# AKGWSB/EzRT

Hardware: NVIDIA H100
Metric: Mrays/s (primary+secondary) (higher is better)
Workload: dtype f32

## Files before the change

ezrt_b200/csrc/device_functions.cuh:

```cuda
#ifndef EZRT_DEVICE_FUNCTIONS_CUH
#define EZRT_DEVICE_FUNCTIONS_CUH

#include "device_scene.h"
#include "ezrt.h"
#include "ezrt_math.h"
#include "w8_node.h"

__constant__ uint32_t c_sobolV[8 * 32] = {
#include "ezrt_sobol_table.inc"
};

typedef ez_vec3 vec3;

__device__ __forceinline__ vec3 f4xyz(float4 q) { return ez_v3(q.x, q.y, q.z); }
__device__ __forceinline__ vec3 splat3(float s) { return ez_v3(s, s, s); }
__device__ __forceinline__ float4 ldg4(const float4* p) { return __ldg(p); }

#ifndef EZRT_MATH_NOINLINE
#define EZRT_MATH_NOINLINE 0
#endif
#if EZRT_MATH_NOINLINE
#define EZD_MATH __device__ __noinline__
#else
#define EZD_MATH __device__ __forceinline__
// ... 711 lines not shown
                        if (strict) {
                            best = tn;
                            best_tri = leaf_first + __ffs(mq) - 1;
                        }
                        if (ANYHIT && (!BOUNDED || strict)) stop = true;
                    }
                    leaf_first += LL;
                    leaf_cnt -= LL;
                }
                if (long_leaves) m_leaf |= __ballot_sync(FULL, pos >= 0 && leaf_cnt > 0 && !stop);
            }
            if (at_leaf) {
                ref = EZRT_REF_DONE;
                if (!stop) {
                    while (sp > 0) {
                        const int2 e = STACK_POP();
                        if (PRUNE && prune_test(__int_as_float(e.y), best, slack)) continue;
                        ref = e.x;
                        break;
                    }
                }
            }
            if (ray >= 0 && ref == EZRT_REF_DONE) {
                HitRec h;
                h.t = best;
                h.tri = best_tri;
                float ix, iy, iz, iz2;
                pk2_split(rs.inv_xy, ix, iy);
                pk2_split(rs.inv_zz, iz, iz2);
                io.store((uint32_t)ray, h, tie, o, d, ez_v3(ix, iy, iz));
                ray = -1;
            }
            busy = __ballot_sync(FULL, ray >= 0);
        } while (busy != 0u && (exhausted || __popc(busy) >= refill_thresh));
    }
    if (COUNT) {
        atomicAdd(counts.node_visits, n_visits);
        atomicAdd(counts.tri_tests, n_tests);
    }
}

#undef STACK_PUSH
#undef STACK_POP

__device__ __forceinline__ uint32_t prmt(uint32_t a, uint32_t b, uint32_t sel) {
    uint32_t r;
    asm("prmt.b32 %0, %1, %2, %3;" : "=r"(r) : "r"(a), "r"(b), "r"(sel));
    return r;
}
template <int K>
__device__ __forceinline__ float w8_plane(uint32_t w, uint32_t bias) {
    uint32_t r;
    asm("prmt.b32 %0, %1, %2, %3;" : "=r"(r) : "r"(w), "r"(bias), "n"(0x7604 | (K << 4)));
    return __uint_as_float(r);
}
template <int K>
__device__ __forceinline__ bool w8_slot_hit(uint32_t nx, uint32_t ny, uint32_t nz, uint32_t fx, uint32_t fy, uint32_t fz, float Bx, float By, float Bz,
                                            float Ax, float Ay, float Az, float limit, uint32_t bias) {
    const float tnx = __fmaf_rn(w8_plane<K>(nx, bias), Bx, Ax), tny = __fmaf_rn(w8_plane<K>(ny, bias), By, Ay), tnz = __fmaf_rn(w8_plane<K>(nz, bias), Bz, Az);
    const float tfx = __fmaf_rn(w8_plane<K>(fx, bias), Bx, Ax), tfy = __fmaf_rn(w8_plane<K>(fy, bias), By, Ay), tfz = __fmaf_rn(w8_plane<K>(fz, bias), Bz, Az);
    const float tmin = fmaxf(fmaxf(tnx, tny), fmaxf(tnz, 0.0f));
    const float tmax = fminf(fminf(tfx, tfy), fminf(tfz, limit));
    return tmin <= tmax;
}

__device__ __forceinline__ int nth_set_bit(uint32_t m, int r) {
    int pos = 0, c = __popc(m & 0xffffu);
    if (r >= c) { r -= c; m >>= 16; pos += 16; }
    c = __popc(m & 0xffu);
    if (r >= c) { r -= c; m >>= 8; pos += 8; }
    c = __popc(m & 0xfu);
    if (r >= c) { r -= c; m >>= 4; pos += 4; }
    c = __popc(m & 0x3u);
    if (r >= c) { r -= c; m >>= 2; pos += 2; }
    return pos + ((r >= (int)(m & 1u)) ? 1 : 0);
}

__device__ __forceinline__ uint32_t w8_clock() {
    uint32_t t;
    asm volatile("mov.u32 %0, %%clock;" : "=r"(t) : : "memory");
    return t;
}

#define W8_ENDED (-2)
template <bool ANYHIT, bool COUNT, bool IDX, bool BOUNDED = false, class RayIO>
__device__ __forceinline__ void extend_w8(const SceneDev& sc, uint32_t n, uint32_t* work, RayIO io, const unsigned char* s_perm, uint2* stack_sm,
                                          W8Counts counts, unsigned long long* phase_cycles) {
    const bool tri_na = sc.tri_l1_bypass != 0;
    const int refill_thresh = sc.refill_thresh, leaf_thresh = sc.w8_tri_weight;
    const unsigned FULL = 0xffffffffu;
    const int lane = threadIdx.x & 31;
    const unsigned lt_mask = (1u << lane) - 1u;
    const int stack_stride = blockDim.x;
    const int stack_cap = sc.w8_stack_entries;
    uint2 stack_local[W8_LOCAL_STACK];
    uint2* const my_stack = stack_sm + threadIdx.x;
    const uint4* __restrict__ nodes = sc.w8_nodes;
    const float origin_limit = sc.w8_origin_limit, inv_limit = sc.quant_inv_limit;
    const uint32_t bias = sc.w8_decode_bits;
    __shared__ unsigned char s_owner_all[EZRT_EXTEND_MAX_THREADS];
    unsigned char* const s_owner = s_owner_all + (threadIdx.x & ~31u);

    int ray = -1;
    int node = -1;
    int end_leaf = 0;
    int sp = 0;
    vec3 o = splat3(0.0f), d = splat3(0.0f), inv = splat3(0.0f);
    float slack = 0.0f, best = EZ_INF;
    int best_tri = -1;
    bool tie = false;
    uint32_t near_mask = 0;
    uint32_t g_base = 0, g_bits = 0;
    uint32_t t_base = 0, t_mask = 0;
    uint32_t n_visits = 0, n_tests = 0;
    uint32_t cyc_refill = 0, cyc_node = 0, cyc_tri = 0, cyc_end = 0;
    uint32_t end_dt = 0, t_mark = COUNT ? w8_clock() : 0u;
    bool exhausted = false;
    uint32_t chunk_pos = 0, chunk_end = 0;
    const uint32_t chunk = (uint32_t)sc.work_chunk;

#define W8_PUSH(e) do { const uint2 e__ = (e); if (sp < stack_cap) my_stack[sp * stack_stride] = e__; else stack_local[sp - stack_cap] = e__; ++sp; } while (0)
#define W8_POP() ((--sp < stack_cap) ? my_stack[sp * stack_stride] : stack_local[sp - stack_cap])
    auto select_next = [&]() {
        if ((g_bits >> 8) == 0u) {
            if (sp == 0) {
                const uint32_t te = COUNT ? w8_clock() : 0u;
                if (best_tri >= 0) end_leaf = io.leaf_of(best_tri);
                if (COUNT) end_dt = w8_clock() - te;
                node = W8_ENDED;
                return;
            }
            const uint2 e = W8_POP();
            g_base = e.x;
            g_bits = e.y;
        }
        const int p = 23 - __clz(g_bits);
        g_bits ^= 0x100u << p;
        const uint32_t slot = (uint32_t)p ^ near_mask;
        node = (int)(g_base + __popc(g_bits & 0xffu & ((1u << slot) - 1u)));
    };

    while (true) {
        const bool ended = node == W8_ENDED;
        const unsigned need = __ballot_sync(FULL, ray < 0 || ended);
        const bool claim = need != 0u && !exhausted && chunk_pos >= chunk_end;
        uint32_t base = 0;
        if (claim && lane == 0) base = atomicAdd(work, chunk);
        if (ended) {
            HitRec h;
            h.t = best;
            h.tri = best_tri;
            const uint32_t te = COUNT ? w8_clock() : 0u;
            io.finish((uint32_t)ray, h, tie, o, d, inv, end_leaf);
            if (COUNT) end_dt = w8_clock() - te;
            ray = -1;
            node = -1;
        }
        if (need != 0u && !exhausted) {
            if (claim) {
                base = __shfl_sync(FULL, base, 0);
                chunk_pos = base;
                chunk_end = (base + chunk < n) ? base + chunk : n;
                if (base >= n) exhausted = true;
            }
            if (!exhausted && ray < 0) {
                uint32_t idx = chunk_pos + (uint32_t)__popc(need & lt_mask);
                if (idx < chunk_end && io.load(idx, o, d)) {
                    inv = ez_v3(EZ_DIV(1.0f, d.x), EZ_DIV(1.0f, d.y), EZ_DIV(1.0f, d.z));
                    const float ax = ez_abs(inv.x), ay = ez_abs(inv.y), az = ez_abs(inv.z);
                    const float ao = fmaxf(ez_abs(o.x), fmaxf(ez_abs(o.y), ez_abs(o.z)));
                    const float amin = fminf(ax, fminf(ay, az)), amax = fmaxf(ax, fmaxf(ay, az));
                    if ((amax <= inv_limit) && (amin >= W8_INV_MIN) && (ao <= origin_limit)) {
                        slack = sc.prune_delta * ez_max(ax, ez_max(ay, az));
                        near_mask = (d.x >= 0.0f ? (1u << sc.w8_near_bit[0]) : 0u) | (d.y >= 0.0f ? (1u << sc.w8_near_bit[1]) : 0u) |
                                    (d.z >= 0.0f ? (1u << sc.w8_near_bit[2]) : 0u);
                        ray = (int)idx;
                        node = 0;
                        sp = 0;
                        g_bits = 0u;
                        t_mask = 0u;
                        best = ray_tmax<BOUNDED>(io, idx);
                        best_tri = -1;
                        tie = false;
                    } else {
                        io.defer(idx, o, d);
                    }
                }
            }
            if (!exhausted) {
                uint32_t take = (uint32_t)__popc(need);
                chunk_pos = (chunk_pos + take < chunk_end) ? chunk_pos + take : chunk_end;
            }
        }
        if (COUNT) {
            const uint32_t now = w8_clock(), e = __reduce_max_sync(FULL, end_dt);
            end_dt = 0u;
            cyc_end += e;
            cyc_refill += now - t_mark - e;
            t_mark = now;
        }
        if (__ballot_sync(FULL, ray >= 0) == 0u) {
            if (exhausted) break;
            continue;
        }
        const int tri_weight = leaf_thresh;
        unsigned busy;
        do {
            const bool at_node = node >= 0;
            const unsigned m_node = __ballot_sync(FULL, at_node);
            const uint32_t pairs = __reduce_add_sync(FULL, (uint32_t)__popc(t_mask));
            if (m_node == 0u && pairs == 0u) { busy = 0u; break; }
            const bool node_step = m_node != 0u && tri_weight * (int)min(pairs, 32u) < __popc(m_node);
            if (node_step) {
                if (at_node) {
                    const uint4* nd = nodes + (size_t)node * (W8_NODE_WORDS / 4);
                    const uint4 h = ldg128_u32(nd), c = ldg128_u32(nd + 1), l = ldg128_u32(nd + 2), m = ldg128_u32(nd + 3), u = ldg128_u32(nd + 4);
                    if (COUNT) n_visits++;
                    const float limit = best + (best * 0.000244140625f + slack);
                    const float Bx = __uint_as_float(W8_SCALE_BITS(h.w, 0)) * inv.x, By = __uint_as_float(W8_SCALE_BITS(h.w, 1)) * inv.y,
                                Bz = __uint_as_float(W8_SCALE_BITS(h.w, 2)) * inv.z;
                    const float Ax = __fmaf_rn(-W8_DECODE_BIAS, Bx, (__uint_as_float(h.x) - o.x) * inv.x);
                    const float Ay = __fmaf_rn(-W8_DECODE_BIAS, By, (__uint_as_float(h.y) - o.y) * inv.y);
                    const float Az = __fmaf_rn(-W8_DECODE_BIAS, Bz, (__uint_as_float(h.z) - o.z) * inv.z);
                    const bool px = d.x >= 0.0f, py = d.y >= 0.0f, pz = d.z >= 0.0f;
                    const uint32_t nx0 = px ? c.z : m.z, nx1 = px ? c.w : m.w, fx0 = px ? m.z : c.z, fx1 = px ? m.w : c.w;
                    const uint32_t ny0 = py ? l.x : u.x, ny1 = py ? l.y : u.y, fy0 = py ? u.x : l.x, fy1 = py ? u.y : l.y;
                    const uint32_t nz0 = pz ? l.z : u.z, nz1 = pz ? l.w : u.w, fz0 = pz ? u.z : l.z, fz1 = pz ? u.w : l.w;
                    uint32_t hits = 0u;
                    if (w8_slot_hit<0>(nx0, ny0, nz0, fx0, fy0, fz0, Bx, By, Bz, Ax, Ay, Az, limit, bias)) hits |= 1u;
                    if (w8_slot_hit<1>(nx0, ny0, nz0, fx0, fy0, fz0, Bx, By, Bz, Ax, Ay, Az, limit, bias)) hits |= 2u;
                    if (w8_slot_hit<2>(nx0, ny0, nz0, fx0, fy0, fz0, Bx, By, Bz, Ax, Ay, Az, limit, bias)) hits |= 4u;
                    if (w8_slot_hit<3>(nx0, ny0, nz0, fx0, fy0, fz0, Bx, By, Bz, Ax, Ay, Az, limit, bias)) hits |= 8u;
                    if (w8_slot_hit<0>(nx1, ny1, nz1, fx1, fy1, fz1, Bx, By, Bz, Ax, Ay, Az, limit, bias)) hits |= 16u;
                    if (w8_slot_hit<1>(nx1, ny1, nz1, fx1, fy1, fz1, Bx, By, Bz, Ax, Ay, Az, limit, bias)) hits |= 32u;
                    if (w8_slot_hit<2>(nx1, ny1, nz1, fx1, fy1, fz1, Bx, By, Bz, Ax, Ay, Az, limit, bias)) hits |= 64u;
                    if (w8_slot_hit<3>(nx1, ny1, nz1, fx1, fy1, fz1, Bx, By, Bz, Ax, Ay, Az, limit, bias)) hits |= 128u;
                    const uint32_t imask = h.w >> 24;
                    const uint32_t inner = hits & imask;
                    uint32_t leaf = hits & ~imask;
                    if ((g_bits >> 8) != 0u) W8_PUSH(make_uint2(g_base, g_bits));
                    g_base = c.x;
                    g_bits = imask | ((uint32_t)s_perm[near_mask * 256u + inner] << 8);
                    t_base = c.y;
                    t_mask = 0u;
                    while (leaf != 0u) {
                        const int s = __ffs(leaf) - 1;
                        leaf &= leaf - 1u;
                        const uint32_t mb = ((s < 4 ? m.x : m.y) >> ((s & 3) * 8)) & 0xffu;
                        t_mask |= ((1u << (mb >> 5)) - 1u) << (mb & 31u);
                    }
                    node = -1;
                    if (t_mask == 0u) select_next();
                }
            } else {
                const uint32_t cnt = (uint32_t)__popc(t_mask);
                uint32_t incl = cnt;
#pragma unroll
                for (int s = 1; s < 32; s <<= 1) {
                    const uint32_t v = __shfl_up_sync(FULL, incl, s);
                    if (lane >= s) incl += v;
                }
                const uint32_t first = incl - cnt;
                const bool owns = cnt != 0u && first < 32u;
                const unsigned starts = __reduce_or_sync(FULL, owns ? 1u << first : 0u);
                __syncwarp();
                if (owns) s_owner[first] = (unsigned char)lane;
                __syncwarp();
                const int start = 31 - __clz(starts & (FULL >> (31 - lane)));
                const bool act = (uint32_t)lane < pairs;
                const int src = act ? (int)s_owner[start] : lane;
                vec3 ro, rd;
                ro.x = __shfl_sync(FULL, o.x, src); ro.y = __shfl_sync(FULL, o.y, src); ro.z = __shfl_sync(FULL, o.z, src);
                rd.x = __shfl_sync(FULL, d.x, src); rd.y = __shfl_sync(FULL, d.y, src); rd.z = __shfl_sync(FULL, d.z, src);
                const float rbest = __shfl_sync(FULL, best, src);
                const uint32_t rmask = __shfl_sync(FULL, t_mask, src);
// ... 843 lines not shown
```

ezrt_b200/csrc/kernels.cu:

```cuda
#include "kernels.h"

#include <cstdlib>
#include <map>
#include <mutex>

#include "device_functions.cuh"

__device__ __forceinline__ void in_tile_xy(int in_tile, int& ix, int& iy) {
    int sub = in_tile >> 5, lane = in_tile & 31;
    ix = (sub & 1) * 8 + (lane & 7);
    iy = (sub >> 1) * 4 + (lane >> 3);
}
__device__ __forceinline__ bool slot_pixel(const RenderDev& rd, const TileDev* __restrict__ tiles, uint32_t slot,
                                           uint32_t& px, uint32_t& py, uint32_t& frame_in_batch) {
    uint32_t per_frame = (uint32_t)rd.n_tiles * EZRT_TILE_PIXELS;
    frame_in_batch = slot / per_frame;
    uint32_t r = slot - frame_in_batch * per_frame;
    TileDev t = tiles[r >> 8];
    int ix, iy;
    in_tile_xy((int)(r & 255u), ix, iy);
    px = (uint32_t)(t.x0 + ix);
    py = (uint32_t)(t.y0 + iy);
    return ix < t.w && iy < t.h;
}
// ... 142 lines not shown
    PathQueue q;
    const uint32_t* perm;
    const uint32_t* to_accel;
    float2* side_hit;
    __device__ __forceinline__ bool load(uint32_t i, vec3& o, vec3& d) const {
        const uint32_t j = perm ? perm[i] : i;
        float4 o4 = __ldcs(q.ray_o + j), d4 = __ldcs(q.ray_d + j);
        o = ez_v3(o4.x, o4.y, o4.z);
        d = ez_v3(d4.x, d4.y, d4.z);
        return true;
    }
    __device__ __forceinline__ void store(uint32_t i, HitRec h, bool, vec3, vec3, vec3) const {
        const uint32_t j = perm ? perm[i] : i;
        int tri = h.tri;
        if (to_accel && tri >= 0) tri = (int)__ldg(to_accel + tri);
        if (side_hit) side_hit[i] = make_float2(h.t, __int_as_float(tri));
        else __stcs(q.hit + j, make_float2(h.t, __int_as_float(tri)));
    }
    __device__ __forceinline__ void defer(uint32_t, vec3, vec3) const {}
};

template <bool PRUNE, bool ANYHIT>
__global__ void __launch_bounds__(EZRT_EXTEND_MAX_THREADS, EZRT_EXTEND_LB_BLOCKS) k_extend(SceneDev sc, PathQueue q, const uint32_t* __restrict__ q_count,
                                                                uint32_t* work, const uint32_t* __restrict__ perm, int to_accel, float2* side_hit, int gate) {
    ExtendIO io;
    io.q = q;
    io.perm = perm;
    io.to_accel = to_accel ? sc.ref_to_acc : nullptr;
    io.side_hit = side_hit;
    const uint32_t n = *q_count;
    if (blockIdx.x * blockDim.x >= n) return;
    if ((gate == 1 && n > EZRT_SIDE_CAP) || (gate == 2 && n <= EZRT_SIDE_CAP)) return;
    TreeView tree = reference_tree(sc);
    if (gate == 1) tree.top_nodes = 0;
    stage_top_nodes(tree);
    extend_persistent<PRUNE, ANYHIT, false, false, 8, false, false>(sc, tree, n, work, io, g_smem_top);
}


struct ShadowIO {
    ShadowQueue sq;
    float4* Lo;
    const uint32_t* perm;
    __device__ __forceinline__ bool load(uint32_t i, vec3& o, vec3& d) const {
        const uint32_t j = perm ? perm[i] : i;
        float4 o4 = __ldcs(sq.ray_o + j), d4 = __ldcs(sq.ray_d + j);
        o = ez_v3(o4.x, o4.y, o4.z);
        d = ez_v3(d4.x, d4.y, d4.z);
        return true;
    }
    __device__ __forceinline__ void mark(uint32_t j, bool lit) const { sq.lit[j] = lit ? 1 : 0; }
    __device__ __forceinline__ float tmax(uint32_t i) const { return __ldcs(sq.nrm + (perm ? perm[i] : i)).w; }
    __device__ __forceinline__ void store(uint32_t i, HitRec h, bool, vec3, vec3, vec3) const { mark(perm ? perm[i] : i, h.tri < 0); }
    __device__ __forceinline__ void defer(uint32_t, vec3, vec3) const {}
};

template <bool PRUNE, bool BOUNDED = false>
__global__ void __launch_bounds__(EZRT_EXTEND_MAX_THREADS, EZRT_EXTEND_LB_BLOCKS) k_shadow(SceneDev sc, ShadowQueue sq, const uint32_t* __restrict__ s_count,
                                                                uint32_t* work, float4* __restrict__ Lo, const uint32_t* __restrict__ perm) {
    ShadowIO io;
    io.sq = sq;
    io.Lo = Lo;
    io.perm = perm;
    const uint32_t n = *s_count;
    if (blockIdx.x * blockDim.x >= n) return;
    const TreeView tree = reference_tree(sc);
    stage_top_nodes(tree);
    extend_persistent<PRUNE, true, false, false, 8, false, false, BOUNDED>(sc, tree, n, work, io, g_smem_top);
}

__device__ __forceinline__ void w8_smem_setup(unsigned char*& s_perm, uint2*& stack_sm) {
    unsigned char* base = reinterpret_cast<unsigned char*>(g_smem_top);
    s_perm = base;
    stack_sm = reinterpret_cast<uint2*>(base + 2048);
    for (int i = threadIdx.x; i < 2048; i += blockDim.x) {
        const int m = i >> 8, x = i & 255;
        int y = 0;
        for (int b = 0; b < 8; b++)
            if ((x >> b) & 1) y |= 1 << (b ^ m);
        s_perm[i] = (unsigned char)y;
    }
    __syncthreads();
}

struct AccelExtendIO {
    PathQueue q;
    const int* acc_tri_leaf;
    const float4* leaf_box;
    uint32_t* defer_list;
    uint32_t* defer_count;
    const uint32_t* perm;
    __device__ __forceinline__ bool load(uint32_t i, vec3& o, vec3& d) const {
        const uint32_t j = perm ? perm[i] : i;
        float4 o4 = __ldcs(q.ray_o + j), d4 = __ldcs(q.ray_d + j);
        o = ez_v3(o4.x, o4.y, o4.z);
        d = ez_v3(d4.x, d4.y, d4.z);
        return true;
    }
    __device__ __forceinline__ void defer(uint32_t i, vec3, vec3) const {
        const uint32_t j = perm ? perm[i] : i;
        __stcs(q.hit + j, make_float2(0.0f, __int_as_float(EZRT_TRI_PENDING)));
        defer_list[atomicAdd(defer_count, 1u)] = j;
    }
    __device__ __forceinline__ void store(uint32_t i, HitRec h, bool tie, vec3 o, vec3 d, vec3 inv) const {
        if (h.tri >= 0 && (tie || !reference_reaches_leaf_inv(acc_tri_leaf, leaf_box, h.tri, o, inv))) {
            defer(i, o, d);
            return;
        }
        __stcs(q.hit + (perm ? perm[i] : i), make_float2(h.t, __int_as_float(h.tri)));
    }
    __device__ __forceinline__ int leaf_of(int tri) const { return __ldg(acc_tri_leaf + tri); }
    __device__ __forceinline__ void finish(uint32_t i, HitRec h, bool tie, vec3 o, vec3 d, vec3 inv, int leaf) const {
        if (h.tri >= 0 && (tie || !reference_reaches_leaf_box(leaf_box, leaf, o, inv))) {
            defer(i, o, d);
            return;
        }
        __stcs(q.hit + (perm ? perm[i] : i), make_float2(h.t, __int_as_float(h.tri)));
    }
};

struct AccelCameraIO {
    RenderDev rd;
    const TileDev* tiles;
    uint32_t batch_first_frame;
    uint32_t n_frames;
    uint32_t per_frame;
    PathQueue q;
    const int* acc_tri_leaf;
    const float4* leaf_box;
    uint32_t* defer_list;
    uint32_t* defer_count;
    __device__ __forceinline__ uint32_t slot_of(uint32_t i) const {
        if (n_frames == 0u) return i;
        const uint32_t p = i / n_frames;
        return (i - p * n_frames) * per_frame + p;
    }
    __device__ __forceinline__ bool load(uint32_t i, vec3& o, vec3& d) const {
        uint32_t px, py, fib, seed;
        if (!slot_pixel(rd, tiles, slot_of(i), px, py, fib)) return false;
        primary_ray(rd, px, py, batch_first_frame + fib, seed, o, d);
        return true;
    }
    __device__ __forceinline__ void defer_slot(uint32_t slot, vec3 o, vec3 d) const {
        q.ray_o[slot] = make_float4(o.x, o.y, o.z, 0.0f);
        q.ray_d[slot] = make_float4(d.x, d.y, d.z, 0.0f);
        __stcs(q.hit + slot, make_float2(0.0f, __int_as_float(EZRT_TRI_PENDING)));
        defer_list[atomicAdd(defer_count, 1u)] = slot;
    }
    __device__ __forceinline__ void defer(uint32_t i, vec3 o, vec3 d) const { defer_slot(slot_of(i), o, d); }
    __device__ __forceinline__ void store(uint32_t i, HitRec h, bool tie, vec3 o, vec3 d, vec3 inv) const {
        const uint32_t slot = slot_of(i);
        if (h.tri >= 0 && (tie || !reference_reaches_leaf_inv(acc_tri_leaf, leaf_box, h.tri, o, inv))) {
            defer_slot(slot, o, d);
            return;
        }
        __stcs(q.hit + slot, make_float2(h.t, __int_as_float(h.tri)));
    }
};

template <bool COUNT, bool IDX>
__global__ void __launch_bounds__(EZRT_EXTEND_MAX_THREADS, EZRT_EXTEND_LB_BLOCKS) k_extend_w8_camera(SceneDev sc, RenderDev rd, const TileDev* __restrict__ tiles,
                                                                   uint32_t batch_first_frame, uint32_t n_slots, uint32_t n_frames, PathQueue q, uint32_t* work,
                                                                   uint32_t* defer_list, uint32_t* defer_count, W8Counts counts) {
    unsigned char* s_perm;
    uint2* stack_sm;
    w8_smem_setup(s_perm, stack_sm);
    AccelCameraIO io;
    io.rd = rd;
    io.tiles = tiles;
    io.batch_first_frame = batch_first_frame;
    io.n_frames = n_frames;
    io.per_frame = (uint32_t)rd.n_tiles * EZRT_TILE_PIXELS;
    io.q = q;
    io.acc_tri_leaf = sc.acc_tri_leaf;
    io.leaf_box = sc.leaf_box;
    io.defer_list = defer_list;
    io.defer_count = defer_count;
    extend_w8_bundle<COUNT, IDX>(sc, n_slots, work, io, s_perm, stack_sm, counts);
}

template <bool COUNT, bool IDX>
__global__ void __launch_bounds__(EZRT_EXTEND_MAX_THREADS, EZRT_EXTEND_LB_BLOCKS) k_extend_w8(SceneDev sc, PathQueue q, const uint32_t* __restrict__ q_count, uint32_t* work,
                                                                   uint32_t* defer_list, uint32_t* defer_count, W8Counts counts, const uint32_t* __restrict__ perm,
                                                                   unsigned long long* phase_cycles) {
    unsigned char* s_perm;
    uint2* stack_sm;
    w8_smem_setup(s_perm, stack_sm);
    AccelExtendIO io;
    io.q = q;
    io.acc_tri_leaf = sc.acc_tri_leaf;
    io.leaf_box = sc.leaf_box;
    io.defer_list = defer_list;
    io.defer_count = defer_count;
    io.perm = perm;
    extend_w8<false, COUNT, IDX>(sc, *q_count, work, io, s_perm, stack_sm, counts, phase_cycles);
}

struct AccelShadowIO {
    ShadowIO base;
    const int* acc_tri_leaf;
    const float4* leaf_box;
    uint32_t* defer_list;
    uint32_t* defer_count;
    __device__ __forceinline__ bool load(uint32_t i, vec3& o, vec3& d) const { return base.load(i, o, d); }
    __device__ __forceinline__ float tmax(uint32_t i) const { return base.tmax(i); }
    __device__ __forceinline__ void defer(uint32_t i, vec3, vec3) const { defer_list[atomicAdd(defer_count, 1u)] = i; }
    __device__ __forceinline__ void store(uint32_t i, HitRec h, bool, vec3 o, vec3 d, vec3 inv) const {
        if (h.tri < 0) {
            base.mark(i, true);
            return;
        }
        if (!reference_reaches_leaf_inv(acc_tri_leaf, leaf_box, h.tri, o, inv)) defer(i, o, d);
        else base.mark(i, false);
    }
    __device__ __forceinline__ int leaf_of(int tri) const { return __ldg(acc_tri_leaf + tri); }
    __device__ __forceinline__ void finish(uint32_t i, HitRec h, bool, vec3 o, vec3 d, vec3 inv, int leaf) const {
        if (h.tri < 0) base.mark(i, true);
        else if (!reference_reaches_leaf_box(leaf_box, leaf, o, inv)) defer(i, o, d);
        else base.mark(i, false);
    }
};

template <bool COUNT, bool IDX, bool BOUNDED = false>
__global__ void __launch_bounds__(EZRT_EXTEND_MAX_THREADS, EZRT_EXTEND_LB_BLOCKS) k_shadow_w8(SceneDev sc, ShadowQueue sq, const uint32_t* __restrict__ s_count, uint32_t* work,
                                                                   float4* __restrict__ Lo, uint32_t* defer_list, uint32_t* defer_count, W8Counts counts,
                                                                   unsigned long long* phase_cycles) {
    unsigned char* s_perm;
    uint2* stack_sm;
    w8_smem_setup(s_perm, stack_sm);
    AccelShadowIO io;
    io.base.sq = sq;
    io.base.Lo = Lo;
    io.base.perm = nullptr;
    io.acc_tri_leaf = sc.acc_tri_leaf;
    io.leaf_box = sc.leaf_box;
    io.defer_list = defer_list;
    io.defer_count = defer_count;
    extend_w8<true, COUNT, IDX, BOUNDED>(sc, *s_count, work, io, s_perm, stack_sm, counts, phase_cycles);
}

template <bool COUNT, bool Q16>
__global__ void __launch_bounds__(EZRT_EXTEND_MAX_THREADS, EZRT_EXTEND_LB_BLOCKS) k_extend_accel(SceneDev sc, PathQueue q, const uint32_t* __restrict__ q_count, uint32_t* work,
                                                                      uint32_t* defer_list, uint32_t* defer_count, W8Counts counts, const uint32_t* __restrict__ perm) {
    AccelExtendIO io;
    io.q = q;
    io.acc_tri_leaf = sc.acc_tri_leaf;
    io.leaf_box = sc.leaf_box;
    io.defer_list = defer_list;
    io.defer_count = defer_count;
    io.perm = perm;
    extend_persistent<true, false, true, true, 4, COUNT, Q16>(sc, accel_tree(sc), *q_count, work, io, g_smem_top, counts);
}
template <bool COUNT>
__global__ void __launch_bounds__(EZRT_EXTEND_MAX_THREADS, EZRT_EXTEND_LB_BLOCKS) k_extend_accel_camera(SceneDev sc, RenderDev rd, const TileDev* __restrict__ tiles,
                                                                      uint32_t batch_first_frame, uint32_t n_slots, uint32_t n_frames, PathQueue q, uint32_t* work,
                                                                      uint32_t* defer_list, uint32_t* defer_count, W8Counts counts) {
    AccelCameraIO io;
    io.rd = rd;
    io.tiles = tiles;
    io.batch_first_frame = batch_first_frame;
    io.n_frames = n_frames;
    io.per_frame = (uint32_t)rd.n_tiles * EZRT_TILE_PIXELS;
    io.q = q;
    io.acc_tri_leaf = sc.acc_tri_leaf;
    io.leaf_box = sc.leaf_box;
    io.defer_list = defer_list;
    io.defer_count = defer_count;
    extend_persistent<true, false, true, true, 4, COUNT, false>(sc, accel_tree(sc), n_slots, work, io, g_smem_top, counts, sc.refill_thresh_camera, sc.work_chunk_camera);
}
template <bool COUNT, bool Q16, bool BOUNDED = false>
__global__ void __launch_bounds__(EZRT_EXTEND_MAX_THREADS, EZRT_EXTEND_LB_BLOCKS) k_shadow_accel(SceneDev sc, ShadowQueue sq, const uint32_t* __restrict__ s_count, uint32_t* work,
                                                                      float4* __restrict__ Lo, uint32_t* defer_list, uint32_t* defer_count, W8Counts counts) {
    AccelShadowIO io;
    io.base.sq = sq;
    io.base.Lo = Lo;
    io.base.perm = nullptr;
    io.acc_tri_leaf = sc.acc_tri_leaf;
    io.leaf_box = sc.leaf_box;
    io.defer_list = defer_list;
    io.defer_count = defer_count;
    extend_persistent<true, true, true, true, 4, COUNT, Q16, BOUNDED>(sc, accel_tree(sc), *s_count, work, io, g_smem_top, counts);
}

#ifndef EZRT_SHADE_REGROUP
#define EZRT_SHADE_REGROUP 0
#endif
#define EZRT_SOBOL_TABLE 256
#define EZRT_SHADE_KEYS 18
#ifndef EZRT_SHADE_PREFETCH
#define EZRT_SHADE_PREFETCH 0
#endif
#ifndef EZRT_SHADE_MIN_BLOCKS
#define EZRT_SHADE_MIN_BLOCKS 8
#endif
template <int MODE, bool LIST, bool AOV = false, bool ENV = false, bool TRANS = false>
__global__ void __launch_bounds__(128, EZRT_SHADE_MIN_BLOCKS) k_shade(SceneDev sc, RenderDev rd, const TileDev* __restrict__ tiles, int bounce,
                                               uint32_t batch_first_frame, PathQueue qin, const uint32_t* __restrict__ in_count,
                                               PathQueue qout, uint32_t* out_count, ShadowQueue sq, uint32_t* s_count,
                                               float4* __restrict__ Lo, float4* __restrict__ Le, uint32_t n_fused, uint32_t n_frames,
                                               const uint32_t* __restrict__ list, const float2* __restrict__ side_hit,
                                               float4* __restrict__ aov_rec, LightsDev lights, EnvDev env) {
    __shared__ float2 s_sobol[EZRT_SOBOL_TABLE];
    const bool sobol_table = (MODE == EZRT_MODE_DISNEY_SOBOL_P5 || MODE == EZRT_MODE_DISNEY_IS_MIS_P5 || MODE == EZRT_MODE_DISNEY_LIGHTS) &&
                             n_frames <= EZRT_SOBOL_TABLE;
    if (sobol_table) {
        for (uint32_t f = threadIdx.x; f < n_frames; f += blockDim.x) s_sobol[f] = sobol_pair(bounce, batch_first_frame + f);
        __syncthreads();
    }
    __shared__ uint32_t s_scan[34];
    const uint32_t n = (LIST || !n_fused) ? *in_count : n_fused;
    if (LIST && n > EZRT_SIDE_CAP) return;
    const uint32_t n_round = ((n + blockDim.x - 1u) / blockDim.x) * blockDim.x;
    const uint32_t stride = gridDim.x * blockDim.x;
#if EZRT_SHADE_REGROUP
    __shared__ float4 s_rg[4][128];
    __shared__ float2 s_rg_hit[128];
    __shared__ unsigned short s_rg_cnt[4][2];
#endif
    for (uint32_t i0 = blockIdx.x * blockDim.x + threadIdx.x; i0 < n_round; i0 += stride) {
        uint32_t i = i0;
#if EZRT_SHADE_PREFETCH
// ... 503 lines not shown
                    const size_t q = (size_t)qy * width + qx;
                    cq = cv_in[q];
                    const float4 aq0 = aov[2 * q];
                    if (aq0.w == 0.0f || !ez_finite(cq.x) || !ez_finite(cq.y) || !ez_finite(cq.z) || !ez_finite(cq.w)) continue;
                    const float4 aq1 = aov[2 * q + 1];
                    const int d = max(abs(i), abs(j));
                    w = ez_atrous_weight(h, (float)(step * d), n_p, ez_v3(aq1.x, aq1.y, aq1.z), ap1.w, aq1.w, Y_p, ez_luminance(ez_v3(cq.x, cq.y, cq.z)),
                                         sd_p, a_p, ez_v3(aq0.x, aq0.y, aq0.z), sigma_l, sigma_n, sigma_z, sigma_a);
                }
                sw = sw + w;
                sc = ez_add(sc, ez_scale(ez_v3(cq.x, cq.y, cq.z), w));
                sv = sv + (w * w) * cq.w;
            }
        }
        res = make_float4(EZ_DIV(sc.x, sw), EZ_DIV(sc.y, sw), EZ_DIV(sc.z, sw), EZ_DIV(sv, sw * sw));
    }
    if (out) {
        const size_t o = p * (size_t)channels;
        if (channels == 4) out[o + 3] = color_in[o + 3];
        out[o] = res.x; out[o + 1] = res.y; out[o + 2] = res.z;
    } else {
        cv_out[p] = res;
    }
}

static inline int div_up(long long a, long long b) { return (int)((a + b - 1) / b); }

static int extend_threads() {
    static int v = 0;
    if (v == 0) {
        v = EZRT_EXTEND_THREADS;
        if (const char* e = getenv("EZRT_EXTEND_THREADS")) v = std::max(32, std::min(EZRT_EXTEND_MAX_THREADS, (atoi(e) / 32) * 32));
    }
    return v;
}
static int extend_blocks_per_sm() {
    static int v = 0;
    if (v == 0) {
        v = EZRT_EXTEND_BLOCKS_PER_SM;
        if (const char* e = getenv("EZRT_EXTEND_BPS")) v = std::max(1, std::min(16, atoi(e)));
    }
    return v;
}
void launch_generate(const RenderDev& rd, const TileDev* tiles, uint32_t n_slots, uint32_t batch_first_frame, PathQueue q,
                     uint32_t* q_count, int n_sms, cudaStream_t st) {
    int blocks = std::min(div_up(n_slots, 256), n_sms * 8);
    k_generate<<<blocks, 256, 0, st>>>(rd, tiles, n_slots, batch_first_frame, q, q_count);
}
static void set_dynamic_smem(const void* kernel, size_t bytes) {
    static std::mutex mu;
    static std::map<const void*, size_t> done;
    std::lock_guard<std::mutex> lock(mu);
    auto it = done.find(kernel);
    if (it != done.end() && it->second >= bytes) return;
    cudaFuncSetAttribute(kernel, cudaFuncAttributeMaxDynamicSharedMemorySize, (int)bytes);
    done[kernel] = bytes;
}
template <class K>
static size_t smem_for(K kernel, int top_nodes) {
    size_t bytes = (size_t)top_nodes * EZRT_TOP_STRIDE * sizeof(float4) + (size_t)EZRT_SMEM_STACK * sizeof(int2) * extend_threads();
    set_dynamic_smem((const void*)kernel, std::max<size_t>(bytes, 1024));
    return bytes;
}
static int persistent_blocks(uint32_t n_max, int n_sms) {
    int blocks = std::min(div_up(n_max, extend_threads()), n_sms * extend_blocks_per_sm());
    return blocks < 1 ? 1 : blocks;
}

void launch_extend(const SceneDev& sc, bool prune, bool anyhit, PathQueue q, const uint32_t* q_count, uint32_t* work,
                   const uint32_t* perm, int to_accel, uint32_t n_max, int n_sms, cudaStream_t st, float2* side_hit, int gate) {
    int threads = extend_threads(), blocks = persistent_blocks(n_max, n_sms);
    int top = sc.top_nodes;
    if (gate == 1) {
        threads = 128;
        blocks = std::max(1, std::min(div_up(n_max, threads), 64));
        top = 0;
    }
    if (prune && anyhit) k_extend<true, true><<<blocks, threads, smem_for(k_extend<true, true>, top), st>>>(sc, q, q_count, work, perm, to_accel, side_hit, gate);
    else if (prune) k_extend<true, false><<<blocks, threads, smem_for(k_extend<true, false>, top), st>>>(sc, q, q_count, work, perm, to_accel, side_hit, gate);
    else if (anyhit) k_extend<false, true><<<blocks, threads, smem_for(k_extend<false, true>, top), st>>>(sc, q, q_count, work, perm, to_accel, side_hit, gate);
    else k_extend<false, false><<<blocks, threads, smem_for(k_extend<false, false>, top), st>>>(sc, q, q_count, work, perm, to_accel, side_hit, gate);
}
template <class K>
static size_t w8_smem_for(K kernel, const SceneDev& sc) {
    size_t bytes = 2048 + (size_t)sc.w8_stack_entries * sizeof(uint2) * extend_threads();
    set_dynamic_smem((const void*)kernel, bytes);
    return bytes;
}
void launch_extend_accel(const SceneDev& sc, PathQueue q, const uint32_t* q_count, uint32_t* work, uint32_t* defer_list,
                         uint32_t* defer_count, uint32_t* defer_work, uint32_t n_max, int n_sms, unsigned long long* counts, const uint32_t* perm,
                         cudaStream_t st, int exact_gate) {
    const int threads = extend_threads(), blocks = persistent_blocks(n_max, n_sms);
    if (sc.w8_nodes) {
        W8Counts c;
        c.node_visits = counts ? counts + 2 : nullptr;
        c.tri_tests = counts ? counts + 1 : nullptr;
        unsigned long long* const cyc = counts ? counts + EZRT_W8_PHASES_EXTEND : nullptr;
#define EZRT_LAUNCH_W8(C, I) k_extend_w8<C, I><<<blocks, threads, w8_smem_for(k_extend_w8<C, I>, sc), st>>>(sc, q, q_count, work, defer_list, defer_count, c, perm, cyc)
        if (sc.acc_tri_indexed) { if (counts) EZRT_LAUNCH_W8(true, true); else EZRT_LAUNCH_W8(false, true); }
        else { if (counts) EZRT_LAUNCH_W8(true, false); else EZRT_LAUNCH_W8(false, false); }
#undef EZRT_LAUNCH_W8
    } else {
        W8Counts c;
        c.node_visits = counts ? (sc.acc_wide_q16 ? counts + 2 : counts) : nullptr;
        c.tri_tests = counts ? counts + 1 : nullptr;
        if (sc.acc_wide_q16) {
            if (counts) k_extend_accel<true, true><<<blocks, threads, smem_for(k_extend_accel<true, true>, 0), st>>>(sc, q, q_count, work, defer_list, defer_count, c, perm);
            else k_extend_accel<false, true><<<blocks, threads, smem_for(k_extend_accel<false, true>, 0), st>>>(sc, q, q_count, work, defer_list, defer_count, c, perm);
        } else {
            if (counts) k_extend_accel<true, false><<<blocks, threads, smem_for(k_extend_accel<true, false>, 0), st>>>(sc, q, q_count, work, defer_list, defer_count, c, perm);
            else k_extend_accel<false, false><<<blocks, threads, smem_for(k_extend_accel<false, false>, 0), st>>>(sc, q, q_count, work, defer_list, defer_count, c, perm);
        }
    }
    launch_extend(sc, true, false, q, defer_count, defer_work, defer_list, 1, std::min<uint32_t>(n_max, 65536u), n_sms, st, nullptr, exact_gate);
}
void launch_ray_sort(const SceneDev& sc, PathQueue q, const uint32_t* q_count, uint32_t* keys, uint32_t* bins, uint32_t* perm,
                     uint32_t n_max, int n_sms, cudaStream_t st) {
    cudaMemsetAsync(bins, 0, sizeof(uint32_t) * EZRT_SORT_BINS, st);
    int blocks = std::max(1, std::min(div_up(n_max, 256), n_sms * 8));
    k_sort_hist<<<blocks, 256, 0, st>>>(sc, q, q_count, keys, bins);
    k_sort_scan<<<1, 1024, 0, st>>>(bins);
    k_sort_scatter<<<blocks, 256, 0, st>>>(q_count, keys, bins, perm);
}
void launch_shadow(const SceneDev& sc, bool prune, ShadowQueue sq, const uint32_t* s_count, uint32_t* work, float4* Lo,
                   const uint32_t* perm, uint32_t n_max, int n_sms, cudaStream_t st, bool bounded) {
    const int threads = extend_threads(), blocks = persistent_blocks(n_max, n_sms);
#define EZRT_LAUNCH_SHADOW(P, B) k_shadow<P, B><<<blocks, threads, smem_for(k_shadow<P, B>, sc.top_nodes), st>>>(sc, sq, s_count, work, Lo, perm)
    if (bounded) { if (prune) EZRT_LAUNCH_SHADOW(true, true); else EZRT_LAUNCH_SHADOW(false, true); }
    else { if (prune) EZRT_LAUNCH_SHADOW(true, false); else EZRT_LAUNCH_SHADOW(false, false); }
#undef EZRT_LAUNCH_SHADOW
}
void launch_extend_camera(const SceneDev& sc, const RenderDev& rd, const TileDev* tiles, uint32_t batch_first_frame, uint32_t n_slots, uint32_t n_frames, PathQueue q,
                          uint32_t* work, uint32_t* defer_list, uint32_t* defer_count, uint32_t* defer_work, int n_sms, unsigned long long* counts,
                          cudaStream_t st, int exact_gate) {
    const int threads = extend_threads(), blocks = persistent_blocks(n_slots, n_sms);
    W8Counts c;
    c.node_visits = counts ? (sc.w8_nodes ? counts + 2 : counts) : nullptr;
    c.tri_tests = counts ? counts + 1 : nullptr;
    if (sc.w8_nodes) {
        auto smem_bundle = [&](const void* k) { const size_t b = 2048 + (size_t)(threads / 32) * W8_BUNDLE_STACK * sizeof(uint2); set_dynamic_smem(k, b); return b; };
#define EZRT_LAUNCH_W8(C, I) \
    k_extend_w8_camera<C, I><<<blocks, threads, smem_bundle((const void*)k_extend_w8_camera<C, I>), st>>>(sc, rd, tiles, batch_first_frame, n_slots, n_frames, q, work, defer_list, defer_count, c)
        if (sc.acc_tri_indexed) { if (counts) EZRT_LAUNCH_W8(true, true); else EZRT_LAUNCH_W8(false, true); }
        else { if (counts) EZRT_LAUNCH_W8(true, false); else EZRT_LAUNCH_W8(false, false); }
#undef EZRT_LAUNCH_W8
    } else {
        if (counts) k_extend_accel_camera<true><<<blocks, threads, smem_for(k_extend_accel_camera<true>, 0), st>>>(sc, rd, tiles, batch_first_frame, n_slots, n_frames, q, work, defer_list, defer_count, c);
        else k_extend_accel_camera<false><<<blocks, threads, smem_for(k_extend_accel_camera<false>, 0), st>>>(sc, rd, tiles, batch_first_frame, n_slots, n_frames, q, work, defer_list, defer_count, c);
    }
    launch_extend(sc, true, false, q, defer_count, defer_work, defer_list, 1, std::min<uint32_t>(n_slots, 65536u), n_sms, st, nullptr, exact_gate);
}
template <bool B>
static void launch_shadow_accel_t(const SceneDev& sc, ShadowQueue sq, const uint32_t* s_count, uint32_t* work, float4* Lo, uint32_t* defer_list,
                                  uint32_t* defer_count, unsigned long long* counts, int blocks, int threads, cudaStream_t st) {
    if (sc.w8_nodes) {
        W8Counts c;
        c.node_visits = counts ? counts + 2 : nullptr;
        c.tri_tests = counts ? counts + 1 : nullptr;
        unsigned long long* const cyc = counts ? counts + EZRT_W8_PHASES_SHADOW : nullptr;
#define EZRT_LAUNCH_W8(C, I) k_shadow_w8<C, I, B><<<blocks, threads, w8_smem_for(k_shadow_w8<C, I, B>, sc), st>>>(sc, sq, s_count, work, Lo, defer_list, defer_count, c, cyc)
        if (sc.acc_tri_indexed) { if (counts) EZRT_LAUNCH_W8(true, true); else EZRT_LAUNCH_W8(false, true); }
        else { if (counts) EZRT_LAUNCH_W8(true, false); else EZRT_LAUNCH_W8(false, false); }
#undef EZRT_LAUNCH_W8
    } else {
        W8Counts c;
        c.node_visits = counts ? (sc.acc_wide_q16 ? counts + 2 : counts) : nullptr;
        c.tri_tests = counts ? counts + 1 : nullptr;
#define EZRT_LAUNCH_W4(C, Q) k_shadow_accel<C, Q, B><<<blocks, threads, smem_for(k_shadow_accel<C, Q, B>, 0), st>>>(sc, sq, s_count, work, Lo, defer_list, defer_count, c)
        if (sc.acc_wide_q16) { if (counts) EZRT_LAUNCH_W4(true, true); else EZRT_LAUNCH_W4(false, true); }
        else { if (counts) EZRT_LAUNCH_W4(true, false); else EZRT_LAUNCH_W4(false, false); }
#undef EZRT_LAUNCH_W4
    }
}
void launch_shadow_accel(const SceneDev& sc, ShadowQueue sq, const uint32_t* s_count, uint32_t* work, float4* Lo, uint32_t* defer_list,
                         uint32_t* defer_count, uint32_t* defer_work, uint32_t n_max, int n_sms, unsigned long long* counts, cudaStream_t st, bool bounded) {
    const int threads = extend_threads(), blocks = persistent_blocks(n_max, n_sms);
    if (bounded) launch_shadow_accel_t<true>(sc, sq, s_count, work, Lo, defer_list, defer_count, counts, blocks, threads, st);
    else launch_shadow_accel_t<false>(sc, sq, s_count, work, Lo, defer_list, defer_count, counts, blocks, threads, st);
    launch_shadow(sc, true, sq, defer_count, defer_work, Lo, defer_list, std::min<uint32_t>(n_max, 65536u), n_sms, st, bounded);
}
void launch_shade(const SceneDev& sc, const RenderDev& rd, const TileDev* tiles, int bounce, uint32_t batch_first_frame,
                  PathQueue qin, const uint32_t* in_count, PathQueue qout, uint32_t* out_count, ShadowQueue sq,
                  uint32_t* s_count, float4* Lo, float4* Le, uint32_t n_max, uint32_t n_fused, uint32_t n_frames, int n_sms, cudaStream_t st,
                  float4* aov_rec, LightsDev lights, EnvDev env, bool trans) {
    int blocks = std::min(div_up(n_max, 128), n_sms * 4 * EZRT_SHADE_MIN_BLOCKS);
    if (blocks < 1) blocks = 1;
#define EZRT_LAUNCH_SHADE_E(M, E, T)                                                                                                          \
    if (aov_rec) k_shade<M, false, true, E, T><<<blocks, 128, 0, st>>>(sc, rd, tiles, bounce, batch_first_frame, qin, in_count, qout, out_count, sq, s_count, Lo, Le, \
                                                                       n_fused, n_frames, nullptr, nullptr, aov_rec, lights, env);           \
    else k_shade<M, false, false, E, T><<<blocks, 128, 0, st>>>(sc, rd, tiles, bounce, batch_first_frame, qin, in_count, qout, out_count, sq, s_count, Lo, Le, n_fused, n_frames, nullptr, nullptr, nullptr, lights, env)
#define EZRT_LAUNCH_SHADE(M) EZRT_LAUNCH_SHADE_E(M, false, false)
    if (rd.mode == EZRT_MODE_DISNEY_LIGHTS && trans) {
        if (env.row_cdf) { EZRT_LAUNCH_SHADE_E(EZRT_MODE_DISNEY_LIGHTS, true, true); }
        else { EZRT_LAUNCH_SHADE_E(EZRT_MODE_DISNEY_LIGHTS, false, true); }
        return;
    }
    if (rd.mode == EZRT_MODE_DISNEY_LIGHTS && env.row_cdf) {
        EZRT_LAUNCH_SHADE_E(EZRT_MODE_DISNEY_LIGHTS, true, false);
        return;
    }
    switch (rd.mode) {
        case EZRT_MODE_DIFFUSE_P3: EZRT_LAUNCH_SHADE(EZRT_MODE_DIFFUSE_P3); break;
        case EZRT_MODE_DISNEY_ANISO_P4: EZRT_LAUNCH_SHADE(EZRT_MODE_DISNEY_ANISO_P4); break;
        case EZRT_MODE_DISNEY_SOBOL_P5: EZRT_LAUNCH_SHADE(EZRT_MODE_DISNEY_SOBOL_P5); break;
        case EZRT_MODE_DISNEY_LIGHTS: EZRT_LAUNCH_SHADE(EZRT_MODE_DISNEY_LIGHTS); break;
        default: EZRT_LAUNCH_SHADE(EZRT_MODE_DISNEY_IS_MIS_P5); break;
    }
#undef EZRT_LAUNCH_SHADE
#undef EZRT_LAUNCH_SHADE_E
}
void launch_deferred_lane(const SceneDev& sc, const RenderDev& rd, const TileDev* tiles, int bounce, uint32_t batch_first_frame, PathQueue qin,
                          const uint32_t* defer_list, const uint32_t* defer_count, uint32_t* defer_work, float2* side_hit, PathQueue qout,
                          uint32_t* out_count, ShadowQueue sq, uint32_t* s_count, float4* Lo, float4* Le, uint32_t n_fused, uint32_t n_frames,
                          int n_sms, cudaStream_t st, float4* aov_rec, LightsDev lights, EnvDev env, bool trans) {
    launch_extend(sc, true, false, qin, defer_count, defer_work, defer_list, 1, EZRT_SIDE_CAP, n_sms, st, side_hit, 1);
    const int blocks = 8;
#define EZRT_LAUNCH_SHADE_E(M, E, T)                                                                                                          \
    if (aov_rec) k_shade<M, true, true, E, T><<<blocks, 128, 0, st>>>(sc, rd, tiles, bounce, batch_first_frame, qin, defer_count, qout, out_count, sq, s_count, Lo, \
                                                                      Le, n_fused, n_frames, defer_list, side_hit, aov_rec, lights, env);      \
    else k_shade<M, true, false, E, T><<<blocks, 128, 0, st>>>(sc, rd, tiles, bounce, batch_first_frame, qin, defer_count, qout, out_count, sq, s_count, Lo, Le, n_fused, n_frames, defer_list, side_hit, nullptr, lights, env)
#define EZRT_LAUNCH_SHADE(M) EZRT_LAUNCH_SHADE_E(M, false, false)
    if (rd.mode == EZRT_MODE_DISNEY_LIGHTS && trans) {
        if (env.row_cdf) { EZRT_LAUNCH_SHADE_E(EZRT_MODE_DISNEY_LIGHTS, true, true); }
        else { EZRT_LAUNCH_SHADE_E(EZRT_MODE_DISNEY_LIGHTS, false, true); }
        return;
    }
    if (rd.mode == EZRT_MODE_DISNEY_LIGHTS && env.row_cdf) {
        EZRT_LAUNCH_SHADE_E(EZRT_MODE_DISNEY_LIGHTS, true, false);
        return;
    }
    switch (rd.mode) {
        case EZRT_MODE_DIFFUSE_P3: EZRT_LAUNCH_SHADE(EZRT_MODE_DIFFUSE_P3); break;
        case EZRT_MODE_DISNEY_ANISO_P4: EZRT_LAUNCH_SHADE(EZRT_MODE_DISNEY_ANISO_P4); break;
        case EZRT_MODE_DISNEY_SOBOL_P5: EZRT_LAUNCH_SHADE(EZRT_MODE_DISNEY_SOBOL_P5); break;
        case EZRT_MODE_DISNEY_LIGHTS: EZRT_LAUNCH_SHADE(EZRT_MODE_DISNEY_LIGHTS); break;
        default: EZRT_LAUNCH_SHADE(EZRT_MODE_DISNEY_IS_MIS_P5); break;
    }
#undef EZRT_LAUNCH_SHADE
#undef EZRT_LAUNCH_SHADE_E
}
void launch_nee(const SceneDev& sc, const RenderDev& rd, ShadowQueue sq, const uint32_t* s_count, float4* Lo, uint32_t n_max, int n_sms, cudaStream_t st,
                bool env, bool trans) {
    const int blocks = std::max(1, std::min(div_up(n_max, 512), n_sms * 8));
// ... 132 lines not shown
```

Baseline: 3333.

## Prefetch next batch of warp rays into shared memory via cp.async double buffering

Replaces per-lane global ray loads at refill time with a per-warp double-buffered shared-memory stage. The next 32 rays (origin, direction, optional tmax) are fetched with cp.async using an L2 evict_first policy, so the fetch overlaps with traversal. Inverse direction and the validity gate are precomputed once per batch and stored in the stage. This adds dynamic shared memory per warp and more complex work-claim bookkeeping, which could reduce occupancy or introduce indexing bugs.

Result: faster. 3371, median of 6 (+1.1%).

```diff
diff --git a/ezrt_b200/csrc/device_functions.cuh b/ezrt_b200/csrc/device_functions.cuh
--- a/ezrt_b200/csrc/device_functions.cuh
+++ b/ezrt_b200/csrc/device_functions.cuh
@@ -817,10 +817,24 @@
     return t;
 }
 
+__device__ __forceinline__ uint64_t l2_evict_first() {
+    uint64_t p;
+    asm volatile("createpolicy.fractional.L2::evict_first.b64 %0, 1.0;" : "=l"(p));
+    return p;
+}
+__device__ __forceinline__ void cp_async16(void* dst, const void* src, uint64_t policy) {
+    asm volatile("cp.async.cg.shared.global.L2::cache_hint [%0], [%1], 16, %2;" : : "r"((uint32_t)__cvta_generic_to_shared(dst)), "l"(src), "l"(policy) : "memory");
+}
+__device__ __forceinline__ void cp_async4(void* dst, const void* src, uint64_t policy) {
+    asm volatile("cp.async.ca.shared.global.L2::cache_hint [%0], [%1], 4, %2;" : : "r"((uint32_t)__cvta_generic_to_shared(dst)), "l"(src), "l"(policy) : "memory");
+}
+__device__ __forceinline__ void cp_async_wait_all() { asm volatile("cp.async.wait_all;" : : : "memory"); }
+
 #define W8_ENDED (-2)
+#define W8_STAGE_BYTES(bounded) (2 * 32 * 32 + 2 * 32 * 4 + ((bounded) ? 2 * 32 * 4 : 0))
 template <bool ANYHIT, bool COUNT, bool IDX, bool BOUNDED = false, class RayIO>
 __device__ __forceinline__ void extend_w8(const SceneDev& sc, uint32_t n, uint32_t* work, RayIO io, const unsigned char* s_perm, uint2* stack_sm,
-                                          W8Counts counts, unsigned long long* phase_cycles) {
+                                          float4* stage_sm, W8Counts counts, unsigned long long* phase_cycles) {
     const bool tri_na = sc.tri_l1_bypass != 0;
     const int refill_thresh = sc.refill_thresh, leaf_thresh = sc.w8_tri_weight;
     const unsigned FULL = 0xffffffffu;
@@ -850,9 +864,56 @@
     uint32_t n_visits = 0, n_tests = 0;
     uint32_t cyc_refill = 0, cyc_node = 0, cyc_tri = 0, cyc_end = 0;
     uint32_t end_dt = 0, t_mark = COUNT ? w8_clock() : 0u;
+
+    __shared__ uint4 s_next_all[EZRT_EXTEND_MAX_THREADS / 32];
+    __shared__ int2 s_cur_all[EZRT_EXTEND_MAX_THREADS / 32];
+    uint4* const s_next = s_next_all + (threadIdx.x >> 5);
+    int2* const s_cur = s_cur_all + (threadIdx.x >> 5);
+    float4* const stage = stage_sm + (threadIdx.x >> 5) * 128;
+    float* const stage_i = reinterpret_cast<float*>(stage_sm + (blockDim.x >> 5) * 128) + (threadIdx.x >> 5) * 64;
+    float* const stage_t = stage_i + (blockDim.x >> 5) * 64;
+    const uint32_t chunk = (uint32_t)sc.work_chunk;
+    uint32_t pos = 0;
+    uint32_t claim = 0;
     bool exhausted = false;
-    uint32_t chunk_pos = 0, chunk_end = 0;
-    const uint32_t chunk = (uint32_t)sc.work_chunk;
+    if (lane == 0) {
+        claim = atomicAdd(work, chunk);
+        *s_next = make_uint4(0u, 0u, 1u, 0u);
+        *s_cur = make_int2(0, 0);
+    }
+    __syncwarp();
+    auto stage_setup = [&](uint32_t b, uint32_t count) {
+        if ((uint32_t)lane < count) {
+            const int k = (int)(b * 32u) + lane;
+            const float4 o4 = stage[k], d4 = stage[64 + k];
+            const float ix = EZ_DIV(1.0f, d4.x), iy = EZ_DIV(1.0f, d4.y), iz = EZ_DIV(1.0f, d4.z);
+            const float ax = ez_abs(ix), ay = ez_abs(iy), az = ez_abs(iz);
+            const float ao = fmaxf(ez_abs(o4.x), fmaxf(ez_abs(o4.y), ez_abs(o4.z)));
+            const float amin = fminf(ax, fminf(ay, az)), amax = fmaxf(ax, fmaxf(ay, az));
+            const bool ok = (amax <= inv_limit) && (amin >= W8_INV_MIN) && (ao <= origin_limit);
+            reinterpret_cast<float*>(stage + k)[3] = ix;
+            reinterpret_cast<float*>(stage + 64 + k)[3] = iy;
+            stage_i[k] = ok ? iz : __int_as_float(0x7fffffff);
+        }
+        __syncwarp();
+    };
+    auto stage_after = [&]() {
+        const uint4 s = *s_next;
+        __syncwarp();
+        uint32_t first = s.x + 32u, end = s.y;
+        if (first >= end) {
+            first = __shfl_sync(FULL, claim, 0);
+            end = min(first + chunk, n);
+            if (lane == 0 && first < n) claim = atomicAdd(work, chunk);
+        }
+        const uint32_t i = first + (uint32_t)lane, k = (s.z ^ 1u) * 32u + (uint32_t)lane;
+        if (i < min(first + 32u, end)) {
+            io.stage(i, stage + k, stage + 64 + k);
+            if constexpr (BOUNDED) io.stage_tmax(i, stage_t + k);
+        }
+        if (lane == 0) *s_next = make_uint4(first, end, s.z ^ 1u, 0u);
+        __syncwarp();
+    };
 
 #define W8_PUSH(e) do { const uint2 e__ = (e); if (sp < stack_cap) my_stack[sp * stack_stride] = e__; else stack_local[sp - stack_cap] = e__; ++sp; } while (0)
 #define W8_POP() ((--sp < stack_cap) ? my_stack[sp * stack_stride] : stack_local[sp - stack_cap])
@@ -878,9 +939,6 @@
     while (true) {
         const bool ended = node == W8_ENDED;
         const unsigned need = __ballot_sync(FULL, ray < 0 || ended);
-        const bool claim = need != 0u && !exhausted && chunk_pos >= chunk_end;
-        uint32_t base = 0;
-        if (claim && lane == 0) base = atomicAdd(work, chunk);
         if (ended) {
             HitRec h;
             h.t = best;
@@ -892,40 +950,55 @@
             node = -1;
         }
         if (need != 0u && !exhausted) {
-            if (claim) {
-                base = __shfl_sync(FULL, base, 0);
-                chunk_pos = base;
-                chunk_end = (base + chunk < n) ? base + chunk : n;
-                if (base >= n) exhausted = true;
-            }
-            if (!exhausted && ray < 0) {
-                uint32_t idx = chunk_pos + (uint32_t)__popc(need & lt_mask);
-                if (idx < chunk_end && io.load(idx, o, d)) {
-                    inv = ez_v3(EZ_DIV(1.0f, d.x), EZ_DIV(1.0f, d.y), EZ_DIV(1.0f, d.z));
-                    const float ax = ez_abs(inv.x), ay = ez_abs(inv.y), az = ez_abs(inv.z);
-                    const float ao = fmaxf(ez_abs(o.x), fmaxf(ez_abs(o.y), ez_abs(o.z)));
-                    const float amin = fminf(ax, fminf(ay, az)), amax = fmaxf(ax, fmaxf(ay, az));
-                    if ((amax <= inv_limit) && (amin >= W8_INV_MIN) && (ao <= origin_limit)) {
-                        slack = sc.prune_delta * ez_max(ax, ez_max(ay, az));
-                        near_mask = (d.x >= 0.0f ? (1u << sc.w8_near_bit[0]) : 0u) | (d.y >= 0.0f ? (1u << sc.w8_near_bit[1]) : 0u) |
-                                    (d.z >= 0.0f ? (1u << sc.w8_near_bit[2]) : 0u);
-                        ray = (int)idx;
-                        node = 0;
-                        sp = 0;
-                        g_bits = 0u;
-                        t_mask = 0u;
-                        best = ray_tmax<BOUNDED>(io, idx);
-                        best_tri = -1;
-                        tie = false;
-                    } else {
-                        io.defer(idx, o, d);
+            const uint32_t r = (uint32_t)__popc(need & lt_mask), take = (uint32_t)__popc(need);
+            int2 cur = *s_cur;
+            const uint32_t avail = (uint32_t)cur.x - pos;
+            uint32_t idx = pos + r;
+            int k = (ray < 0 && r < avail) ? cur.y + (int)idx : -1;
+            const bool advance = take >= avail;
+            if (!advance) {
+                pos += take;
+            } else {
+                cp_async_wait_all();
+                __syncwarp();
+                const uint4 s = *s_next;
+                pos = s.x;
+                cur = make_int2((int)min(s.x + 32u, s.y), (int)(s.z * 32u) - (int)s.x);
+                if (lane == 0) *s_cur = cur;
+                if (s.x >= n) {
+                    exhausted = true;
+                } else {
+                    stage_setup(s.z, (uint32_t)cur.x - s.x);
+                    if (ray < 0 && r >= avail && pos + (r - avail) < (uint32_t)cur.x) {
+                        idx = pos + (r - avail);
+                        k = cur.y + (int)idx;
                     }
+                    pos = min(pos + (take - avail), (uint32_t)cur.x);
                 }
             }
-            if (!exhausted) {
-                uint32_t take = (uint32_t)__popc(need);
-                chunk_pos = (chunk_pos + take < chunk_end) ? chunk_pos + take : chunk_end;
-            }
+            if (k >= 0) {
+                const float4 o4 = stage[k], d4 = stage[64 + k];
+                const float iz = stage_i[k];
+                o = ez_v3(o4.x, o4.y, o4.z);
+                d = ez_v3(d4.x, d4.y, d4.z);
+                if (iz == iz) {
+                    inv = ez_v3(o4.w, d4.w, iz);
+                    slack = sc.prune_delta * ez_max(ez_abs(inv.x), ez_max(ez_abs(inv.y), ez_abs(inv.z)));
+                    near_mask = (d.x >= 0.0f ? (1u << sc.w8_near_bit[0]) : 0u) | (d.y >= 0.0f ? (1u << sc.w8_near_bit[1]) : 0u) |
+                                (d.z >= 0.0f ? (1u << sc.w8_near_bit[2]) : 0u);
+                    ray = (int)idx;
+                    node = 0;
+                    sp = 0;
+                    g_bits = 0u;
+                    t_mask = 0u;
+                    best = BOUNDED ? stage_t[k] : EZ_INF;
+                    best_tri = -1;
+                    tie = false;
+                } else {
+                    io.defer(idx, o, d);
+                }
+            }
+            if (advance && !exhausted) stage_after();
         }
         if (COUNT) {
             const uint32_t now = w8_clock(), e = __reduce_max_sync(FULL, end_dt);
diff --git a/ezrt_b200/csrc/kernels.cu b/ezrt_b200/csrc/kernels.cu
--- a/ezrt_b200/csrc/kernels.cu
+++ b/ezrt_b200/csrc/kernels.cu
@@ -248,6 +248,9 @@
     }
     __syncthreads();
 }
+__device__ __forceinline__ float4* w8_stage_smem(const SceneDev& sc, uint2* stack_sm) {
+    return reinterpret_cast<float4*>(stack_sm + (size_t)sc.w8_stack_entries * blockDim.x);
+}
 
 struct AccelExtendIO {
     PathQueue q;
@@ -274,6 +277,12 @@
             return;
         }
         __stcs(q.hit + (perm ? perm[i] : i), make_float2(h.t, __int_as_float(h.tri)));
+    }
+    __device__ __forceinline__ void stage(uint32_t i, float4* o, float4* d) const {
+        const uint32_t j = perm ? perm[i] : i;
+        const uint64_t pol = l2_evict_first();
+        cp_async16(o, q.ray_o + j, pol);
+        cp_async16(d, q.ray_d + j, pol);
     }
     __device__ __forceinline__ int leaf_of(int tri) const { return __ldg(acc_tri_leaf + tri); }
     __device__ __forceinline__ void finish(uint32_t i, HitRec h, bool tie, vec3 o, vec3 d, vec3 inv, int leaf) const {
@@ -359,7 +368,7 @@
     io.defer_list = defer_list;
     io.defer_count = defer_count;
     io.perm = perm;
-    extend_w8<false, COUNT, IDX>(sc, *q_count, work, io, s_perm, stack_sm, counts, phase_cycles);
+    extend_w8<false, COUNT, IDX>(sc, *q_count, work, io, s_perm, stack_sm, w8_stage_smem(sc, stack_sm), counts, phase_cycles);
 }
 
 struct AccelShadowIO {
@@ -370,6 +379,12 @@
     uint32_t* defer_count;
     __device__ __forceinline__ bool load(uint32_t i, vec3& o, vec3& d) const { return base.load(i, o, d); }
     __device__ __forceinline__ float tmax(uint32_t i) const { return base.tmax(i); }
+    __device__ __forceinline__ void stage(uint32_t i, float4* o, float4* d) const {
+        const uint64_t pol = l2_evict_first();
+        cp_async16(o, base.sq.ray_o + i, pol);
+        cp_async16(d, base.sq.ray_d + i, pol);
+    }
+    __device__ __forceinline__ void stage_tmax(uint32_t i, float* t) const { cp_async4(t, &base.sq.nrm[i].w, l2_evict_first()); }
     __device__ __forceinline__ void defer(uint32_t i, vec3, vec3) const { defer_list[atomicAdd(defer_count, 1u)] = i; }
     __device__ __forceinline__ void store(uint32_t i, HitRec h, bool, vec3 o, vec3 d, vec3 inv) const {
         if (h.tri < 0) {
@@ -402,7 +417,7 @@
     io.leaf_box = sc.leaf_box;
     io.defer_list = defer_list;
     io.defer_count = defer_count;
-    extend_w8<true, COUNT, IDX, BOUNDED>(sc, *s_count, work, io, s_perm, stack_sm, counts, phase_cycles);
+    extend_w8<true, COUNT, IDX, BOUNDED>(sc, *s_count, work, io, s_perm, stack_sm, w8_stage_smem(sc, stack_sm), counts, phase_cycles);
 }
 
 template <bool COUNT, bool Q16>
@@ -1072,8 +1087,8 @@
     else k_extend<false, false><<<blocks, threads, smem_for(k_extend<false, false>, top), st>>>(sc, q, q_count, work, perm, to_accel, side_hit, gate);
 }
 template <class K>
-static size_t w8_smem_for(K kernel, const SceneDev& sc) {
-    size_t bytes = 2048 + (size_t)sc.w8_stack_entries * sizeof(uint2) * extend_threads();
+static size_t w8_smem_for(K kernel, const SceneDev& sc, bool bounded) {
+    size_t bytes = 2048 + (size_t)sc.w8_stack_entries * sizeof(uint2) * extend_threads() + (size_t)(extend_threads() / 32) * W8_STAGE_BYTES(bounded);
     set_dynamic_smem((const void*)kernel, bytes);
     return bytes;
 }
@@ -1086,7 +1101,7 @@
         c.node_visits = counts ? counts + 2 : nullptr;
         c.tri_tests = counts ? counts + 1 : nullptr;
         unsigned long long* const cyc = counts ? counts + EZRT_W8_PHASES_EXTEND : nullptr;
-#define EZRT_LAUNCH_W8(C, I) k_extend_w8<C, I><<<blocks, threads, w8_smem_for(k_extend_w8<C, I>, sc), st>>>(sc, q, q_count, work, defer_list, defer_count, c, perm, cyc)
+#define EZRT_LAUNCH_W8(C, I) k_extend_w8<C, I><<<blocks, threads, w8_smem_for(k_extend_w8<C, I>, sc, false), st>>>(sc, q, q_count, work, defer_list, defer_count, c, perm, cyc)
         if (sc.acc_tri_indexed) { if (counts) EZRT_LAUNCH_W8(true, true); else EZRT_LAUNCH_W8(false, true); }
         else { if (counts) EZRT_LAUNCH_W8(true, false); else EZRT_LAUNCH_W8(false, false); }
 #undef EZRT_LAUNCH_W8
@@ -1148,7 +1163,7 @@
         c.node_visits = counts ? counts + 2 : nullptr;
         c.tri_tests = counts ? counts + 1 : nullptr;
         unsigned long long* const cyc = counts ? counts + EZRT_W8_PHASES_SHADOW : nullptr;
-#define EZRT_LAUNCH_W8(C, I) k_shadow_w8<C, I, B><<<blocks, threads, w8_smem_for(k_shadow_w8<C, I, B>, sc), st>>>(sc, sq, s_count, work, Lo, defer_list, defer_count, c, cyc)
+#define EZRT_LAUNCH_W8(C, I) k_shadow_w8<C, I, B><<<blocks, threads, w8_smem_for(k_shadow_w8<C, I, B>, sc, B), st>>>(sc, sq, s_count, work, Lo, defer_list, defer_count, c, cyc)
         if (sc.acc_tri_indexed) { if (counts) EZRT_LAUNCH_W8(true, true); else EZRT_LAUNCH_W8(false, true); }
         else { if (counts) EZRT_LAUNCH_W8(true, false); else EZRT_LAUNCH_W8(false, false); }
 #undef EZRT_LAUNCH_W8
```
